# NVIDIA/MinkowskiEngine

Measured on AMD Instinct MI355X. Metric: MinkowskiConvolution fwd+bwd Mpoints/sec (100k-pt 3D, k=3), higher is better.
Workload: dtype f32

## Files before the change

minkowskiengine_amd/csrc/conv.hip:

```cpp
#include "conv_common.hpp"
#include "wgrad_reduce.hpp"

#include <algorithm>
#include <type_traits>
#include <vector>

namespace me {

__host__ __device__ constexpr int stage_ld(int kc) {
  return kc == 96 ? 100 : (kc >= 32 ? kc : kc + 4);
}
__device__ __forceinline__ int stage_swz(int kc, int row) {
  return kc == 96 ? 0 : (kc >= 64 ? (row & 15) : (kc == 32 ? ((row >> 1) & 7) : 0));
}

__host__ __device__ constexpr int conv_lds_bytes(int nc, int kc, int tile_rows, int batch_groups) {
  return (tile_rows + 1) * (nc + kAccPad) * 4 + batch_groups * 16 * (stage_ld(kc) * 4 + 4);
}

template <int R, int KQ, int A_LD, int ACC_LD, int VAR = 0>
__device__ __forceinline__ void mma_groups(const float *__restrict__ a0p, const int (&pofs)[KQ / 4],
                                           const float (&wreg)[KQ], const int32_t *__restrict__ dstp,
                                           float *__restrict__ accp) {
  int d[R];
// ... 1263 lines not shown
  __syncthreads();                                   \
  cm = cw;
    for (;;) {
      ME_WG_STEP(1)
      ME_WG_STEP(2)
      ME_WG_STEP(3)
      ME_WG_STEP(0)
    }
#undef ME_WG_STEP
  } else {
    __builtin_amdgcn_s_setprio(2);
    const int i16 = lane & 15, q = lane >> 4;
    const int cob = blockIdx.z * 4 + wave;
    constexpr int kImage = MB * NB * 4 * 64;
    const int64_t image_stride = (int64_t)gridDim.y * n_cob * kImage;
    float *const image0 = partial + ((int64_t)blockIdx.y * n_cob + min(cob, n_cob - 1)) * kImage + lane;
    f32x4 acc[MB][NB];
    auto zero_acc = [&]() {
#pragma unroll
      for (int m = 0; m < MB; ++m)
#pragma unroll
        for (int n = 0; n < NB; ++n) acc[m][n] = f32x4{0.f, 0.f, 0.f, 0.f};
    };
    auto flush = [&](int k) {
      if (cob < n_cob) {
        float *img = image0 + (int64_t)(range + k) * image_stride;
#pragma unroll
        for (int m = 0; m < MB; ++m)
#pragma unroll
          for (int n = 0; n < NB; ++n)
#pragma unroll
            for (int r = 0; r < 4; ++r) img[((m * NB + n) * 4 + r) * 64] = acc[m][n][r];
      }
    };
    const int frag_row = 4 * q + (i16 >> 2);
    const int frag_col = 4 * (i16 & 3);
    auto multiply = [&](int buf) {
      const __bf16 *bx = s_x + (buf * SP + frag_row) * XLD + frag_col;
      const __bf16 *bd = s_d + (buf * SP + frag_row) * DLD + wave * 16 * NB + frag_col;
#pragma unroll
      for (int ks = 0; ks < KSTEPS; ++ks) {
        bf16x8 a[MB], b[NB];
#pragma unroll
        for (int m = 0; m < MB; ++m) {
          const bf16x4 lo = __builtin_amdgcn_ds_read_tr16_b64_v4bf16((lds_bf16x4 *)(bx + (ks * 32) * XLD + 16 * m));
          const bf16x4 hi = __builtin_amdgcn_ds_read_tr16_b64_v4bf16((lds_bf16x4 *)(bx + (ks * 32 + 16) * XLD + 16 * m));
          a[m] = bf16x8{lo[0], lo[1], lo[2], lo[3], hi[0], hi[1], hi[2], hi[3]};
        }
#pragma unroll
        for (int n = 0; n < NB; ++n) {
          const bf16x4 lo = __builtin_amdgcn_ds_read_tr16_b64_v4bf16((lds_bf16x4 *)(bd + (ks * 32) * DLD + 16 * n));
          const bf16x4 hi = __builtin_amdgcn_ds_read_tr16_b64_v4bf16((lds_bf16x4 *)(bd + (ks * 32 + 16) * DLD + 16 * n));
          b[n] = bf16x8{lo[0], lo[1], lo[2], lo[3], hi[0], hi[1], hi[2], hi[3]};
        }
#pragma unroll
        for (int m = 0; m < MB; ++m)
#pragma unroll
          for (int n = 0; n < NB; ++n) acc[m][n] = __builtin_amdgcn_mfma_f32_16x16x32_bf16(a[m], b[n], acc[m][n], 0, 0, 0);
      }
    };
    Cur cA = first_cur();
    Cur cB = next_cur(cA);
    zero_acc();
    __syncthreads();
    int buf = 0;
    while (cA.cnt > 0) {
      multiply(buf);
      if (cB.cnt == 0 || cB.k != cA.k) {
        flush(cA.k);
        zero_acc();
      }
      __syncthreads();
      buf ^= 1;
      cA = cB;
      cB = next_cur(cB);
    }
    __builtin_amdgcn_s_setprio(0);
  }
}

#endif

template <int NB>
__global__ __launch_bounds__(256, 3) void k_wgrad_f32x3(const float *__restrict__ x, int c_in,
                                                       const float *__restrict__ dy, int c_out,
                                                       const int32_t *__restrict__ in_pairs,
                                                       const int32_t *__restrict__ out_pairs,
                                                       const int64_t *__restrict__ koffs, int volume,
                                                       int64_t n_pairs, int n_ranges, int n_cob,
                                                       float *__restrict__ partial, const WgRangeOrder order) {
  typedef __attribute__((address_space(3))) bf16x4 lds_bf16x4;
  constexpr int MB = 4;
  constexpr int SP = 32;
  constexpr int COB = 64 * NB;
  constexpr int XLD = 64 + kWgStepLd;
  constexpr int DLD = COB + kWgStepLd;
  constexpr int XPL = SP * XLD, DPL = SP * DLD;
  constexpr int XP = SP * 8 / 256;
  constexpr int DP = SP * (COB / 8) / 256;
  static_assert(XP == 1 && DP >= 1, "step size");
  extern __shared__ __attribute__((aligned(16))) char smem[];
  __bf16 *s_x = reinterpret_cast<__bf16 *>(smem);
  __bf16 *s_d = s_x + 3 * XPL;

  const int tid = threadIdx.x;
  const int lane = tid & 63;
  const int wave = __builtin_amdgcn_readfirstlane(tid >> 6);
  const int i16 = lane & 15, q = lane >> 4;
  const int range = order.n > 0 ? (int)order.v[blockIdx.x] : (int)blockIdx.x;
  const int ci0 = blockIdx.y * 64;
  const int cog = blockIdx.z * COB;
  const int cob = blockIdx.z * 4 + wave;
  const int64_t e_lo = n_pairs * range / n_ranges;
  const int64_t e_hi = n_pairs * (range + 1) / n_ranges;
  if (e_lo >= e_hi) return;

  constexpr int kImage = MB * NB * 4 * 64;
  const int64_t image_stride = (int64_t)gridDim.y * n_cob * kImage;
  float *const image0 = partial + ((int64_t)blockIdx.y * n_cob + min(cob, n_cob - 1)) * kImage + lane;

  auto first_offset = [&](int64_t e) {
    int lo = 0, hi = volume;
    while (hi - lo > 1) {
      const int mid = (lo + hi) >> 1;
      if (koffs[mid] <= e) lo = mid; else hi = mid;
    }
    return lo;
  };
  auto step_count = [&](int k, int64_t e) -> int {
    if (e >= e_hi) return 0;
    const int64_t kend = min(koffs[k + 1], e_hi);
    return (int)min((int64_t)SP, kend - e);
  };
  auto advance = [&](int &k, int64_t &e, int cnt) {
    e += cnt;
    if (e < e_hi) {
      while (koffs[k + 1] <= e) ++k;
    }
  };

  int32_t pin = 0, pout = 0;
  f32x4 rx[XP][2], rd[DP][2];
  auto load_idx = [&](int64_t e) {
    const int64_t ec = min(e + lane, n_pairs - 1);
    const int32_t *pi = in_pairs + ec, *po = out_pairs + ec;
    asm volatile("global_load_dword %0, %1, off" : "=v"(pin) : "v"(pi) : "memory");
    asm volatile("global_load_dword %0, %1, off" : "=v"(pout) : "v"(po) : "memory");
  };
  auto load_rows = [&]() {
#pragma unroll
    for (int j = 0; j < XP; ++j) {
      const int idx = j * 256 + tid;
      const int row = idx >> 3;
      const int ch = ci0 + (idx & 7) * 8;
      const int32_t r = __shfl(pin, row, 64);
      const float *p = x + (int64_t)r * c_in + (ch < c_in ? ch : 0);
      asm volatile("global_load_dwordx4 %0, %1, off" : "=v"(rx[j][0]) : "v"(p) : "memory");
      asm volatile("global_load_dwordx4 %0, %1, off offset:16" : "=v"(rx[j][1]) : "v"(p) : "memory");
    }
#pragma unroll
    for (int j = 0; j < DP; ++j) {
      const int idx = j * 256 + tid;
      const int row = idx / (COB / 8);
      const int ch = cog + (idx % (COB / 8)) * 8;
      const int32_t r = __shfl(pout, row, 64);
      const float *p = dy + (int64_t)r * c_out + (ch < c_out ? ch : 0);
      asm volatile("global_load_dwordx4 %0, %1, off" : "=v"(rd[j][0]) : "v"(p) : "memory");
      asm volatile("global_load_dwordx4 %0, %1, off offset:16" : "=v"(rd[j][1]) : "v"(p) : "memory");
    }
  };
  auto wait_rows = [&]() {
    asm volatile("s_waitcnt vmcnt(0)" : "+v"(pin), "+v"(pout));
#pragma unroll
// ... 43 lines not shown
  };

  f32x4 acc[MB][NB];
  auto zero_acc = [&]() {
#pragma unroll
    for (int m = 0; m < MB; ++m)
#pragma unroll
      for (int n = 0; n < NB; ++n) acc[m][n] = f32x4{0.f, 0.f, 0.f, 0.f};
  };
  auto flush = [&](int k) {
    if (cob < n_cob) {
      float *img = image0 + (int64_t)(range + k) * image_stride;
#pragma unroll
      for (int m = 0; m < MB; ++m)
#pragma unroll
        for (int n = 0; n < NB; ++n)
#pragma unroll
          for (int r = 0; r < 4; ++r) img[((m * NB + n) * 4 + r) * 64] = acc[m][n][r];
    }
  };
  const int frag_row = 4 * q + (i16 >> 2);
  const int frag_col = 4 * (i16 & 3);
  auto multiply = [&]() {
    const __bf16 *bx = s_x + frag_row * XLD + frag_col;
    const __bf16 *bd = s_d + frag_row * DLD + wave * 16 * NB + frag_col;
    bf16x8 a[3][MB], b[3][NB];
#pragma unroll
    for (int pl = 0; pl < 3; ++pl) {
#pragma unroll
      for (int m = 0; m < MB; ++m) {
        const bf16x4 lo = __builtin_amdgcn_ds_read_tr16_b64_v4bf16((lds_bf16x4 *)(bx + pl * XPL + 16 * m));
        const bf16x4 hi = __builtin_amdgcn_ds_read_tr16_b64_v4bf16((lds_bf16x4 *)(bx + pl * XPL + 16 * XLD + 16 * m));
        a[pl][m] = bf16x8{lo[0], lo[1], lo[2], lo[3], hi[0], hi[1], hi[2], hi[3]};
      }
#pragma unroll
      for (int n = 0; n < NB; ++n) {
        const bf16x4 lo = __builtin_amdgcn_ds_read_tr16_b64_v4bf16((lds_bf16x4 *)(bd + pl * DPL + 16 * n));
        const bf16x4 hi = __builtin_amdgcn_ds_read_tr16_b64_v4bf16((lds_bf16x4 *)(bd + pl * DPL + 16 * DLD + 16 * n));
        b[pl][n] = bf16x8{lo[0], lo[1], lo[2], lo[3], hi[0], hi[1], hi[2], hi[3]};
      }
    }
    constexpr int XPI[6] = {2, 0, 1, 1, 0, 0};
    constexpr int DPI[6] = {0, 2, 1, 0, 1, 0};
#pragma unroll
    for (int t = 0; t < 6; ++t)
#pragma unroll
      for (int m = 0; m < MB; ++m)
#pragma unroll
        for (int n = 0; n < NB; ++n)
          acc[m][n] = __builtin_amdgcn_mfma_f32_16x16x32_bf16(a[XPI[t]][m], b[DPI[t]][n], acc[m][n], 0, 0, 0);
  };

  int kA = first_offset(e_lo);
  int64_t eA = e_lo;
  int cA = step_count(kA, eA);
  int kB = kA;
  int64_t eB = eA;
  advance(kB, eB, cA);
  int cB = step_count(kB, eB);
  int kC = kB;
  int64_t eC = eB;
  advance(kC, eC, cB);
  int cC = step_count(kC, eC);

  load_idx(eA);
  asm volatile("s_waitcnt vmcnt(0)" : "+v"(pin), "+v"(pout));
  load_rows();
  load_idx(eB);
  zero_acc();
  int pending = -1;
  while (cA > 0) {
    if (pending >= 0) {
      flush(pending);
      zero_acc();
    }
    wait_rows();
    __syncthreads();
    write_lds(cA);
    load_rows();
    load_idx(eC);
    __builtin_amdgcn_sched_barrier(0);
    __syncthreads();
    multiply();
    pending = (cB == 0 || kB != kA) ? kA : -1;
    kA = kB; eA = eB; cA = cB;
    kB = kC; eB = eC; cB = cC;
    advance(kC, eC, cC);
    cC = step_count(kC, eC);
  }
  wait_rows();
  if (pending >= 0) flush(pending);
}

#ifdef ME_DEBUG_VARIANTS
template <int NB, int KSTEPS>
__global__ __launch_bounds__(256, 2) void k_wgrad_lds_f32(const float *__restrict__ x, int c_in,
                                                         const float *__restrict__ dy, int c_out,
                                                      const int32_t *__restrict__ in_pairs,
                                                      const int32_t *__restrict__ out_pairs,
                                                      const int64_t *__restrict__ koffs, int volume,
                                                      int64_t n_pairs, int n_ranges, int n_cob,
                                                      float *__restrict__ partial) {
  constexpr int MB = 4;
  constexpr int SP = 16 * KSTEPS;
  constexpr int COB = 64 * NB;
  constexpr int XLD = 64 + kWgStepLd;
  constexpr int DLD = COB + kWgStepLd;
  constexpr int XP = SP * 16 / 256;
  constexpr int DP = SP * (COB / 4) / 256;
  static_assert(SP <= 64 && XP >= 1, "step size");
  extern __shared__ __attribute__((aligned(16))) char smem[];
  float *s_x = reinterpret_cast<float *>(smem);
  float *s_d = s_x + 2 * SP * XLD;

  const int tid = threadIdx.x;
  const int lane = tid & 63;
  const int wave = __builtin_amdgcn_readfirstlane(tid >> 6);
  const int i16 = lane & 15, q = lane >> 4;
  const int range = blockIdx.x;
  const int ci0 = blockIdx.y * 64;
  const int cog = blockIdx.z * COB;
  const int cob = blockIdx.z * 4 + wave;
  const int64_t e_lo = n_pairs * range / n_ranges;
  const int64_t e_hi = n_pairs * (range + 1) / n_ranges;
  if (e_lo >= e_hi) return;

  constexpr int kImage = MB * NB * 4 * 64;
  const int64_t image_stride = (int64_t)gridDim.y * n_cob * kImage;
  float *const image0 = partial + ((int64_t)blockIdx.y * n_cob + min(cob, n_cob - 1)) * kImage + lane;

  auto first_offset = [&](int64_t e) {
    int lo = 0, hi = volume;
    while (hi - lo > 1) {
      const int mid = (lo + hi) >> 1;
      if (koffs[mid] <= e) lo = mid; else hi = mid;
    }
    return lo;
  };
  auto step_count = [&](int k, int64_t e) -> int {
    if (e >= e_hi) return 0;
    const int64_t kend = min(koffs[k + 1], e_hi);
    return (int)min((int64_t)SP, kend - e);
  };
  auto advance = [&](int &k, int64_t &e, int cnt) {
    e += cnt;
    if (e < e_hi) {
      while (koffs[k + 1] <= e) ++k;
    }
  };

  int32_t pin = 0, pout = 0;
  f32x4 rx[XP], rd[DP];
  auto load_idx = [&](int64_t e) {
    const int64_t ec = min(e + lane, n_pairs - 1);
    const int32_t *pi = in_pairs + ec, *po = out_pairs + ec;
    asm volatile("global_load_dword %0, %1, off" : "=v"(pin) : "v"(pi) : "memory");
    asm volatile("global_load_dword %0, %1, off" : "=v"(pout) : "v"(po) : "memory");
  };
  auto load_rows = [&]() {
#pragma unroll
    for (int j = 0; j < XP; ++j) {
      const int idx = j * 256 + tid;
      const int row = idx >> 4;
      const int ch = ci0 + (idx & 15) * 4;
      const int32_t r = __shfl(pin, row, 64);
      const float *p = x + (int64_t)r * c_in + (ch < c_in ? ch : 0);
// ... 260 lines not shown
                            const int32_t *plan_src, const int32_t *plan_dst, const int32_t *batch_desc,
                            const int32_t *tile_bptr, const int32_t *order, float *dst, int64_t n_tgt,
                            int tile_rows, int batch_groups, hipStream_t stream, bool small = false, bool fuse = false) {
  const int lds = conv_lds_bytes(NC, KC, tile_rows, batch_groups) +
                  (g_conv_variant >= 2048 && g_conv_variant < 3000 ? (g_conv_variant - 2048) * 1024 : 0);
  ME_CHECK(lds <= kLdsBudget, "tile_rows / batch_groups too large for the LDS of one workgroup");
  const bool exact = (c_src % KC) == 0;
  constexpr bool kHasSmall = VAR == 0;
  small = small && kHasSmall;
  typedef void (*kernel_t)(const float *, int, const f32x4 *, int, const int32_t *, const int32_t *, const int32_t *,
                           const int32_t *, const int32_t *, float *, int64_t, int, int);
  kernel_t fn = (small && exact) ? &k_conv_tile_f32<NC, KC, true, VAR, kHasSmall> : &k_conv_tile_f32<NC, KC, false, VAR, false>;
  constexpr bool kHasFuse = VAR == 0 && NC <= 64 && KC <= 64;
  if constexpr (kHasFuse) {
    if (fuse && small) fn = exact ? &k_conv_tile_f32<NC, KC, true, 0, true, true> : &k_conv_tile_f32<NC, KC, false, 0, true, true>;
    else fuse = false;
  } else {
    fuse = false;
  }
  static bool attr_set[6] = {false, false, false, false, false, false};
  const int which = fuse ? 4 + (exact ? 1 : 0) : (small ? 2 : 0) + (exact ? 1 : 0);
  if (lds > 48 * 1024 && !attr_set[which]) {
    ME_HIP(hipFuncSetAttribute(reinterpret_cast<const void *>(fn), hipFuncAttributeMaxDynamicSharedMemorySize,
                               kLdsBudget));
    attr_set[which] = true;
  }
  const dim3 grid((unsigned)ceil_div(n_tgt, tile_rows), (unsigned)slabs);
  hipLaunchKernelGGL(fn, grid, dim3(NC * 4), (size_t)lds, stream, src, c_src, reinterpret_cast<const f32x4 *>(wp), c_dst,
                     plan_src, plan_dst, batch_desc, tile_bptr, order, dst, n_tgt, tile_rows, batch_groups);
  ME_LAUNCH_CHECK();
  return 0;
}

template <int NC, int CBW, int KCH>
static int launch_conv_tile_dma(const float *src, int c_src, const float *wp, int c_dst, const int32_t *plan_src,
                                const int32_t *plan_dst, const int32_t *batch_desc, const int32_t *tile_bptr,
                                const int32_t *order, float *dst, int64_t n_tgt, int tile_rows, int batch_groups,
                                hipStream_t stream) {
  const int lds = conv_dma_lds_bytes(NC, KCH, tile_rows, batch_groups);
  ME_CHECK(lds <= kLdsBudget, "tile_rows / batch_groups too large for the LDS of one workgroup (LDS-DMA kernel)");
  typedef void (*kernel_t)(const float *, int, const f32x4 *, int, const int32_t *, const int32_t *, const int32_t *,
                           const int32_t *, const int32_t *, float *, int64_t, int, int);
  kernel_t fn = &k_conv_tile_dma_f32<NC, CBW, KCH, 0>;
  const int code = g_conv_variant % 100;
  if (code == 16) fn = &k_conv_tile_dma_f32<NC, CBW, KCH, 16>;
  if constexpr (NC == 128 && CBW == 2) {
    if (code == 2) fn = &k_conv_tile_dma_f32<NC, CBW, KCH, 2>;
    if (code == 4) fn = &k_conv_tile_dma_f32<NC, CBW, KCH, 4>;
    if (code == 32) fn = &k_conv_tile_dma_f32<NC, CBW, KCH, 32>;
    if (code == 64) fn = &k_conv_tile_dma_f32<NC, CBW, KCH, 64>;
    if (code == 99) fn = &k_conv_tile_dma_f32<NC, CBW, KCH, 16 + 2 + 4 + 32 + 64>;
    if (code == 98) fn = &k_conv_tile_dma_f32<NC, CBW, KCH, 512>;
  }
  ME_HIP(hipFuncSetAttribute(reinterpret_cast<const void *>(fn), hipFuncAttributeMaxDynamicSharedMemorySize,
                             kLdsBudget));
  const dim3 grid((unsigned)ceil_div(n_tgt, tile_rows), (unsigned)(c_dst / NC));
  hipLaunchKernelGGL(fn, grid, dim3(NC / CBW * 4), (size_t)lds, stream, src, c_src,
                     reinterpret_cast<const f32x4 *>(wp), c_dst, plan_src, plan_dst, batch_desc, tile_bptr, order, dst,
                     n_tgt, tile_rows, batch_groups);
  ME_LAUNCH_CHECK();
  return 0;
}

struct ConvDmaShape {
  int nc, cbw, kch;
};
static ConvDmaShape conv_dma_shape(int c_src, int c_dst) {
  ConvDmaShape z{0, 0, 0};
  if (g_conv_variant < 3000 || g_conv_variant >= 3400) return z;
  if (c_src % 64 != 0 || c_dst % 64 != 0) return z;
  const int family = g_conv_variant / 100;
  if (family == 30) {
    if (g_conv_variant == 3064) return ConvDmaShape{64, 1, 1};
    return c_dst % 128 == 0 ? ConvDmaShape{128, 1, 1} : ConvDmaShape{64, 1, 1};
  }
  if (c_dst % 128 == 0) return ConvDmaShape{128, 2, 1};
  if (c_src % 128 == 0) return ConvDmaShape{64, 1, 2};
  return ConvDmaShape{64, 1, 1};
}

int g_wgrad_depth = 0;
int g_wgrad_wgs_per_cu = 0;
int g_wgrad_order = 0;

struct WgradGeom {
  int nb;
  int n_cib;
  int n_cob;
  int waves;
  int gz;
  int64_t ranges;
  int64_t slot_floats;
};

static WgradGeom wgrad_geom(int64_t n_pairs, int64_t volume, int c_in, int c_out) {
  WgradGeom g;
  g.nb = c_out <= 64 ? 1 : (c_out <= 128 ? 2 : 4);
  if (g_wgrad_depth >= 100) g.nb = g_wgrad_depth / 100;
  g.n_cib = (int)ceil_div(c_in, 16 * kWgMB);
  g.n_cob = (int)ceil_div(c_out, 16 * g.nb);
  g.waves = g.n_cob < 4 ? g.n_cob : 4;
  g.gz = (int)ceil_div(g.n_cob, g.waves);
  const int wpc = g_wgrad_wgs_per_cu > 0 ? g_wgrad_wgs_per_cu : 3;
  int64_t r = ceil_div((int64_t)device_cu_count() * wpc, (int64_t)g.n_cib * g.gz);
  if (r > n_pairs / 64) r = n_pairs / 64;
  if (r < 1) r = 1;
  g.ranges = r;
  g.slot_floats = (int64_t)g.n_cib * g.n_cob * (kWgMB * g.nb * 4 * 64);
  (void)volume;
  return g;
}

int g_wgrad_ws = 0;
int g_wgrad_mb = 0;

static int wgrad_bf16_mb(int c_in, int c_out) {
  if (g_wgrad_mb == 4 || g_wgrad_mb == 8) return (g_wgrad_mb == 8 && c_out > 64) ? 8 : 4;
  return (c_in >= 192 && c_out > 64) ? 8 : 4;
}

static WgradGeom wgrad_geom_staged(int64_t n_pairs, int c_in, int c_out, int wpc_default = 2, int mb = kWgMB) {
  WgradGeom g;
  g.nb = c_out <= 64 ? 1 : 2;
  g.n_cib = (int)ceil_div(c_in, 16 * mb);
  g.n_cob = (int)ceil_div(c_out, 16 * g.nb);
  g.waves = 4;
  g.gz = (int)ceil_div(g.n_cob, 4);
  const int wpc = g_wgrad_wgs_per_cu > 0 ? g_wgrad_wgs_per_cu : (g.n_cib == 3 ? 3 : wpc_default);
  int64_t r = ceil_div((int64_t)device_cu_count() * wpc, (int64_t)g.n_cib * g.gz);
  if (r > n_pairs / 64) r = n_pairs / 64;
  if (r < 1) r = 1;
  g.ranges = r;
  g.slot_floats = (int64_t)g.n_cib * g.n_cob * (mb * g.nb * 4 * 64);
  return g;
}

template <int NB, int KSTEPS, int MB = kWgMB>
static int launch_wgrad_bf16(const WgradGeom &g, const __bf16 *x, int c_in, const __bf16 *dy, int c_out,
                             const int32_t *in_pairs, const int32_t *out_pairs, const int64_t *k_offsets_dev,
                             int volume, int64_t n_pairs, float *partial, hipStream_t stream) {
  constexpr int SP = 32 * KSTEPS;
  const int lds = 2 * SP * ((16 * MB + kWgStepLd) + (64 * NB + kWgStepLd)) * 2;
  auto fn = &k_wgrad_bf16<NB, KSTEPS, MB>;
  static bool attr_set = false;
  if (lds > 32 * 1024 && !attr_set) {
    ME_HIP(hipFuncSetAttribute(reinterpret_cast<const void *>(fn), hipFuncAttributeMaxDynamicSharedMemorySize,
                               kLdsBudget));
    attr_set = true;
  }
  const dim3 grid((unsigned)g.ranges, (unsigned)g.n_cib, (unsigned)g.gz);
#ifdef ME_DEBUG_VARIANTS
  if (g_wgrad_ws != 0) {
    auto ws = g_wgrad_ws == 2 ? &k_wgrad_bf16_ws<NB, KSTEPS, MB, 2> : &k_wgrad_bf16_ws<NB, KSTEPS, MB, (MB == 8 ? 2 : 4)>;
    static bool ws_attr[2] = {false, false};
    if (lds > 32 * 1024 && !ws_attr[g_wgrad_ws == 2]) {
      ME_HIP(hipFuncSetAttribute(reinterpret_cast<const void *>(ws), hipFuncAttributeMaxDynamicSharedMemorySize, kLdsBudget));
      ws_attr[g_wgrad_ws == 2] = true;
    }
    hipLaunchKernelGGL(ws, grid, dim3(512), (size_t)lds, stream, x, c_in, dy, c_out, in_pairs, out_pairs, k_offsets_dev,
                       volume, n_pairs, (int)g.ranges, g.n_cob, partial);
    ME_LAUNCH_CHECK();
    return 0;
  }
#endif
  hipLaunchKernelGGL(fn, grid, dim3(256), (size_t)lds, stream, x, c_in, dy, c_out, in_pairs,
                     out_pairs, k_offsets_dev, volume, n_pairs, (int)g.ranges, g.n_cob, partial);
  ME_LAUNCH_CHECK();
  return 0;
}

#ifdef ME_DEBUG_VARIANTS
template <int NB, int KSTEPS>
static int launch_wgrad_lds_f32(const WgradGeom &g, const float *x, int c_in, const float *dy, int c_out,
                                const int32_t *in_pairs, const int32_t *out_pairs, const int64_t *k_offsets_dev,
                                int volume, int64_t n_pairs, float *partial, hipStream_t stream) {
  constexpr int SP = 16 * KSTEPS;
  const int lds = 2 * SP * ((64 + kWgStepLd) + (64 * NB + kWgStepLd)) * 4;
  static bool attr_set = false;
  if (lds > 32 * 1024 && !attr_set) {
    ME_HIP(hipFuncSetAttribute(reinterpret_cast<const void *>(&k_wgrad_lds_f32<NB, KSTEPS>),
                               hipFuncAttributeMaxDynamicSharedMemorySize, kLdsBudget));
    attr_set = true;
  }
  const dim3 grid((unsigned)g.ranges, (unsigned)g.n_cib, (unsigned)g.gz);
  hipLaunchKernelGGL((k_wgrad_lds_f32<NB, KSTEPS>), grid, dim3(256), (size_t)lds, stream, x, c_in, dy, c_out,
                     in_pairs, out_pairs, k_offsets_dev, volume, n_pairs, (int)g.ranges, g.n_cob, partial);
  ME_LAUNCH_CHECK();
  return 0;
}
#endif

template <int NB>
static int launch_wgrad_f32x3(const WgradGeom &g, const float *x, int c_in, const float *dy, int c_out,
                              const int32_t *in_pairs, const int32_t *out_pairs, const int64_t *k_offsets_dev,
                              int volume, int64_t n_pairs, float *partial, const WgRangeOrder &order,
                              hipStream_t stream) {
  const int lds = 3 * 32 * ((64 + kWgStepLd) + (64 * NB + kWgStepLd)) * 2;
  const dim3 grid((unsigned)g.ranges, (unsigned)g.n_cib, (unsigned)g.gz);
  hipLaunchKernelGGL((k_wgrad_f32x3<NB>), grid, dim3(256), (size_t)lds, stream, x, c_in, dy, c_out, in_pairs,
                     out_pairs, k_offsets_dev, volume, n_pairs, (int)g.ranges, g.n_cob, partial, order);
  ME_LAUNCH_CHECK();
  return 0;
}

static bool wgrad_use_split(int c_in, int c_out) {
  if (g_wgrad_depth == -3 || (c_in % 8) != 0 || (c_out % 8) != 0) return false;
  if (g_wgrad_depth == -4) return true;
  return g_wgrad_depth == 0 && c_in >= 32 && c_out >= 32;
}

bool wgrad_split_tail(const int64_t *k_offsets, const int64_t *k_offsets_dev, int64_t volume, int c_in, int c_out,
                      const void *workspace, float *grad_w, WgTail *tail) {
  if (!wgrad_use_split(c_in, c_out) || volume < 1 || volume > 65535) return false;
  const int64_t n_pairs = k_offsets[volume];
  const WgradGeom g = wgrad_geom_staged(n_pairs, c_in, c_out, 3);
  tail->r = WgReduceArgs{reinterpret_cast<const float *>(workspace), k_offsets_dev, grad_w, n_pairs > 0 ? n_pairs : 1,
                         (int)volume, (int)g.ranges, g.n_cib, g.n_cob, c_in, c_out};
  tail->nb = g.nb;
  tail->n_tiles = 0;
  return true;
}

}

using namespace me;

static WgRangeOrder wgrad_range_order(const int64_t *k_offsets, int64_t volume, int64_t n_pairs, int64_t ranges,
                                      int64_t wgs_per_range) {
  WgRangeOrder o;
  o.n = 0;
  if (g_wgrad_order < 0 || ranges < 64 || ranges > kWgMaxOrder || wgs_per_range != 1 || volume < 2) return o;
  struct Item {
    double f;
    int r;
  };
  std::vector<Item> items((size_t)ranges);
  int k = 0;
  for (int64_t r = 0; r < ranges; ++r) {
    const int64_t e = wgrad_range_begin(r, n_pairs, ranges);
    while (k + 1 < volume && k_offsets[k + 1] <= e) ++k;
    const int64_t len = k_offsets[k + 1] - k_offsets[k];
    items[(size_t)r] = {len > 0 ? (double)(e - k_offsets[k]) / (double)len : 0.0, (int)r};
  }
  std::stable_sort(items.begin(), items.end(), [](const Item &a, const Item &b) { return a.f < b.f; });
  constexpr int kXcds = 8, kGroup = 32;
  std::vector<std::vector<int>> per_xcd(kXcds);
  for (int64_t i = 0; i < ranges; ++i) per_xcd[(size_t)((i / kGroup) % kXcds)].push_back(items[(size_t)i].r);
  std::vector<int> assigned((size_t)ranges, -1), spill;
  for (int x = 0; x < kXcds; ++x) {
    for (size_t i = 0; i < per_xcd[(size_t)x].size(); ++i) {
      const int64_t b = (int64_t)i * kXcds + x;
      if (b < ranges) assigned[(size_t)b] = per_xcd[(size_t)x][i];
      else spill.push_back(per_xcd[(size_t)x][i]);
    }
  }
  size_t sp = 0;
  for (int64_t b = 0; b < ranges; ++b)
    if (assigned[(size_t)b] < 0) assigned[(size_t)b] = spill[sp++];
  o.n = (int)ranges;
  for (int64_t b = 0; b < ranges; ++b) o.v[b] = (uint16_t)assigned[(size_t)b];
  return o;
}

template <typename T>
static int wgrad_launch(const T *x, int64_t n_in, int32_t c_in, const T *dy, int64_t n_out, int32_t c_out,
                        const int32_t *in_pairs, const int32_t *out_pairs, const int64_t *k_offsets,
                        const int64_t *k_offsets_dev, int64_t volume, float *grad_w, void *workspace,
                        int64_t workspace_bytes, hipStream_t stream) {
  ME_CHECK(volume >= 1 && volume <= 65535, "kernel volume out of range");
  ME_CHECK(c_in > 0 && c_out > 0, "channel counts must be positive");
  ME_CHECK((uintptr_t)x % 16 == 0 && (uintptr_t)dy % 16 == 0, "feature pointers must be 16-byte aligned");
  ME_CHECK(workspace_bytes >= me_conv_wgrad_workspace_bytes(k_offsets, volume, c_in, c_out),
           "workspace too small");
  const int64_t n_pairs = k_offsets[volume];
  const WgradGeom g = wgrad_geom(n_pairs, volume, c_in, c_out);
  float *partial = reinterpret_cast<float *>(workspace);
  const int depth = (g_wgrad_depth > 0 && g_wgrad_depth % 100 > 0) ? g_wgrad_depth % 100 : (g.nb == 4 ? 8 : 4);
  if (n_pairs > 0) {
    const dim3 grid((unsigned)g.ranges, (unsigned)g.n_cib, (unsigned)g.gz);
    const dim3 block(64 * g.waves);
    const bool vec = (c_in % kWgMB) == 0 && (c_out % g.nb) == 0;
    const int64_t lim = 1ll << 32;
    const bool small = n_in > 0 && n_out > 0 && n_in < (1 << 24) && n_out < (1 << 24) &&
                       n_in * c_in * (int64_t)sizeof(T) < lim && n_out * c_out * (int64_t)sizeof(T) < lim &&
                       g_conv_variant != 6;
    const WgRangeOrder order = wgrad_range_order(k_offsets, volume, n_pairs, g.ranges, (int64_t)g.n_cib * g.gz);
#define ME_WGRAD_LAUNCH(NBV, DV)                                                                                 \
  do {                                                                                                           \
    if (vec && small)                                                                                            \
      hipLaunchKernelGGL((k_wgrad_f32<T, NBV, DV, true, true>), grid, block, 0, stream, x, c_in, dy, c_out,      \
                         in_pairs, out_pairs, k_offsets_dev, (int)volume, n_pairs, (int)g.ranges, g.n_cob,       \
// ... 138 lines not shown
    if (v.kc == 96) ME_CONV_CASE(64, 96);
    if (v.kc == 64) ME_CONV_CASE(64, 64);
    if (v.kc == 32) ME_CONV_CASE(64, 32);
    ME_CONV_CASE(64, 16);
  }
#undef ME_CONV_CASE
#undef ME_CONV_ARGS
}

int me_conv_target_f32(const float *src, int64_t n_src, int32_t c_src, const float *wp, int64_t volume,
                       int32_t c_dst, const int32_t *plan_src, const int32_t *plan_dst,
                       const int32_t *batch_desc, const int32_t *tile_bptr, const int32_t *order, float *dst,
                       int64_t n_tgt, int32_t tile_rows, int32_t batch_groups, void *stream) {
  return conv_target_f32(src, n_src, c_src, wp, volume, c_dst, plan_src, plan_dst, batch_desc, tile_bptr, order, dst,
                         n_tgt, tile_rows, batch_groups, stream, false);
}

int me_conv_target_f32_fused(const float *src, int64_t n_src, int32_t c_src, const float *wp, int64_t volume,
                             int32_t c_dst, const int32_t *plan_src, const int32_t *plan_dst,
                             const int32_t *batch_desc, const int32_t *tile_bptr, const int32_t *order, float *dst,
                             int64_t n_tgt, int32_t tile_rows, int32_t batch_groups, void *stream) {
  return conv_target_f32(src, n_src, c_src, wp, volume, c_dst, plan_src, plan_dst, batch_desc, tile_bptr, order, dst,
                         n_tgt, tile_rows, batch_groups, stream, true);
}

int32_t me_debug_variants_compiled(void) {
#ifdef ME_DEBUG_VARIANTS
  return 1;
#else
  return 0;
#endif
}

int me_debug_set_conv_variant(int variant) {
#ifndef ME_DEBUG_VARIANTS
  const bool ok = variant == 0 || variant == 6 || variant == 7 || variant == 9 || variant == 30 || variant == 31;
  ME_CHECK(ok, "this conv variant needs a -DME_DEBUG_VARIANTS build of libme_amd.so (tuning / ablation kernels)");
#endif
  g_conv_variant = variant;
  return 0;
}

int me_debug_conv_timing(uint64_t *out8, int32_t reset) {
  unsigned long long h[8] = {0, 0, 0, 0, 0, 0, 0, 0};
  if (out8 != nullptr) {
    ME_HIP(hipMemcpyFromSymbol(h, HIP_SYMBOL(d_conv_timing), sizeof(h)));
    for (int i = 0; i < 8; ++i) out8[i] = h[i];
  }
  if (reset) {
    unsigned long long z[8] = {0, 0, 0, 0, 0, 0, 0, 0};
    ME_HIP(hipMemcpyToSymbol(HIP_SYMBOL(d_conv_timing), z, sizeof(z)));
  }
  return 0;
}


int me_transpose_kernel_f32(const float *w, int64_t volume, int32_t c_in, int32_t c_out, float *wt,
                            void *stream_) {
  hipStream_t stream = (hipStream_t)stream_;
  ME_CHECK(volume >= 1 && volume <= 65535, "kernel volume out of range");
  const dim3 grid((unsigned)ceil_div(c_out, 32), (unsigned)ceil_div(c_in, 32), (unsigned)volume);
  hipLaunchKernelGGL(k_transpose_kernel, grid, dim3(256), 0, stream, w, volume, c_in, c_out, wt);
  ME_LAUNCH_CHECK();
  return 0;
}

int64_t me_conv_wgrad_workspace_bytes(const int64_t *k_offsets, int64_t volume, int32_t c_in, int32_t c_out) {
  if (volume < 1 || c_in <= 0 || c_out <= 0) return 256;
  const WgradGeom g = wgrad_geom(k_offsets[volume], volume, c_in, c_out);
  const WgradGeom h = wgrad_geom_staged(k_offsets[volume], c_in, c_out, 3);
  const int64_t a = (g.ranges + volume) * g.slot_floats, b = (h.ranges + volume) * h.slot_floats;
  return align_up((a > b ? a : b) * 4, 256);
}

void me_debug_set_wgrad_order(int mode) { g_wgrad_order = mode; }
void me_debug_set_wgrad_mb(int mb) { g_wgrad_mb = mb; }
void me_debug_set_wgrad_ws(int mode) { g_wgrad_ws = mode; }

void me_debug_set_wgrad_config(int depth, int wgs_per_cu) {
  g_wgrad_depth = depth;
  g_wgrad_wgs_per_cu = wgs_per_cu;
}

static int wgrad_split_partials(const float *x, int32_t c_in, const float *dy, int32_t c_out, const int32_t *in_pairs,
                                const int32_t *out_pairs, const int64_t *k_offsets, const int64_t *k_offsets_dev,
                                int64_t volume, void *workspace, int64_t workspace_bytes, hipStream_t stream,
                                WgradGeom *geom) {
  ME_CHECK(volume >= 1 && volume <= 65535, "kernel volume out of range");
  ME_CHECK((uintptr_t)x % 16 == 0 && (uintptr_t)dy % 16 == 0, "feature pointers must be 16-byte aligned");
  ME_CHECK(workspace_bytes >= me_conv_wgrad_workspace_bytes(k_offsets, volume, c_in, c_out), "workspace too small");
  const int64_t n_pairs = k_offsets[volume];
  const WgradGeom g = wgrad_geom_staged(n_pairs, c_in, c_out, 3);
  float *partial = reinterpret_cast<float *>(workspace);
  *geom = g;
  if (n_pairs <= 0) return 0;
  const WgRangeOrder order = wgrad_range_order(k_offsets, volume, n_pairs, g.ranges, (int64_t)g.n_cib * g.gz);
  return g.nb == 1 ? launch_wgrad_f32x3<1>(g, x, c_in, dy, c_out, in_pairs, out_pairs, k_offsets_dev, (int)volume,
                                           n_pairs, partial, order, stream)
                   : launch_wgrad_f32x3<2>(g, x, c_in, dy, c_out, in_pairs, out_pairs, k_offsets_dev, (int)volume,
                                           n_pairs, partial, order, stream);
}

int32_t me_conv_wgrad_is_split_f32(int32_t c_in, int32_t c_out) { return wgrad_use_split(c_in, c_out) ? 1 : 0; }

int me_conv_wgrad_partials_f32(const float *x, int64_t n_in, int32_t c_in, const float *dy, int64_t n_out, int32_t c_out,
                               const int32_t *in_pairs, const int32_t *out_pairs, const int64_t *k_offsets,
                               const int64_t *k_offsets_dev, int64_t volume, void *workspace, int64_t workspace_bytes,
                               void *stream_) {
  (void)n_in;
  (void)n_out;
  ME_CHECK(wgrad_use_split(c_in, c_out), "not a split weight gradient (me_conv_wgrad_is_split_f32)");
  WgradGeom g;
  return wgrad_split_partials(x, c_in, dy, c_out, in_pairs, out_pairs, k_offsets, k_offsets_dev, volume, workspace,
                              workspace_bytes, (hipStream_t)stream_, &g);
}

int me_conv_wgrad_f32(const float *x, int64_t n_in, int32_t c_in, const float *dy, int64_t n_out, int32_t c_out,
                      const int32_t *in_pairs,
                      const int32_t *out_pairs, const int64_t *k_offsets, const int64_t *k_offsets_dev,
                      int64_t volume, float *grad_w, void *workspace, int64_t workspace_bytes,
                      void *stream_) {
  hipStream_t stream = (hipStream_t)stream_;
  if (wgrad_use_split(c_in, c_out)) {
    WgradGeom g;
    const int rc = wgrad_split_partials(x, c_in, dy, c_out, in_pairs, out_pairs, k_offsets, k_offsets_dev, volume,
                                        workspace, workspace_bytes, stream, &g);
    if (rc != 0) return rc;
    const float *partial = reinterpret_cast<const float *>(workspace);
    const int64_t n_pairs = k_offsets[volume];
    const dim3 rgrid((unsigned)ceil_div(g.slot_floats, 256), (unsigned)volume);
    if (g.nb == 1)
      hipLaunchKernelGGL((k_wgrad_reduce<1, true>), rgrid, dim3(64 * kWgReducePhases), 0, stream, partial, k_offsets_dev,
                         (int)volume, n_pairs > 0 ? n_pairs : 1, (int)g.ranges, g.n_cib, g.n_cob, c_in, c_out, grad_w);
    else
      hipLaunchKernelGGL((k_wgrad_reduce<2, true>), rgrid, dim3(64 * kWgReducePhases), 0, stream, partial, k_offsets_dev,
                         (int)volume, n_pairs > 0 ? n_pairs : 1, (int)g.ranges, g.n_cib, g.n_cob, c_in, c_out, grad_w);
    ME_LAUNCH_CHECK();
    return 0;
  }
#ifndef ME_DEBUG_VARIANTS
  return wgrad_launch<float>(x, n_in, c_in, dy, n_out, c_out, in_pairs, out_pairs, k_offsets, k_offsets_dev, volume, grad_w,
                             workspace, workspace_bytes, stream);
#else
  if ((c_in % 4) != 0 || (c_out % 4) != 0 || g_wgrad_depth != -2)
    return wgrad_launch<float>(x, n_in, c_in, dy, n_out, c_out, in_pairs, out_pairs, k_offsets, k_offsets_dev, volume, grad_w,
                               workspace, workspace_bytes, stream);
  ME_CHECK(volume >= 1 && volume <= 65535, "kernel volume out of range");
  ME_CHECK(c_in > 0 && c_out > 0, "channel counts must be positive");
  ME_CHECK((uintptr_t)x % 16 == 0 && (uintptr_t)dy % 16 == 0, "feature pointers must be 16-byte aligned");
  ME_CHECK(workspace_bytes >= me_conv_wgrad_workspace_bytes(k_offsets, volume, c_in, c_out), "workspace too small");
  const int64_t n_pairs = k_offsets[volume];
  const WgradGeom g = wgrad_geom_staged(n_pairs, c_in, c_out);
  float *partial = reinterpret_cast<float *>(workspace);
  if (n_pairs > 0) {
    int rc;
    if (g.nb == 1)
      rc = launch_wgrad_lds_f32<1, 2>(g, x, c_in, dy, c_out, in_pairs, out_pairs, k_offsets_dev, (int)volume, n_pairs,
                                      partial, stream);
    else
      rc = launch_wgrad_lds_f32<2, 2>(g, x, c_in, dy, c_out, in_pairs, out_pairs, k_offsets_dev, (int)volume, n_pairs,
                                      partial, stream);
    if (rc != 0) return rc;
  }
  const dim3 rgrid((unsigned)ceil_div(g.slot_floats, 256), (unsigned)volume);
  if (g.nb == 1)
    hipLaunchKernelGGL((k_wgrad_reduce<1, true>), rgrid, dim3(64 * kWgReducePhases), 0, stream, partial, k_offsets_dev, (int)volume,
                       n_pairs > 0 ? n_pairs : 1, (int)g.ranges, g.n_cib, g.n_cob, c_in, c_out, grad_w);
  else
    hipLaunchKernelGGL((k_wgrad_reduce<2, true>), rgrid, dim3(64 * kWgReducePhases), 0, stream, partial, k_offsets_dev, (int)volume,
                       n_pairs > 0 ? n_pairs : 1, (int)g.ranges, g.n_cib, g.n_cob, c_in, c_out, grad_w);
  ME_LAUNCH_CHECK();
  return 0;
#endif
}

}

extern "C" {

int64_t me_conv_wgrad_workspace_bytes_bf16(const int64_t *k_offsets, int64_t volume, int32_t c_in, int32_t c_out) {
  if (volume < 1 || c_in <= 0 || c_out <= 0) return 256;
  const WgradGeom g4 = wgrad_geom_staged(k_offsets[volume], c_in, c_out, 2, 4);
  const WgradGeom g8 = wgrad_geom_staged(k_offsets[volume], c_in, c_out, 2, 8);
  const int64_t a4 = align_up((g4.ranges + volume) * g4.slot_floats * 4, 256);
  const int64_t a8 = align_up((g8.ranges + volume) * g8.slot_floats * 4, 256);
  const int64_t a = a4 > a8 ? a4 : a8;
  const int64_t b = me_conv_wgrad_workspace_bytes(k_offsets, volume, c_in, c_out);
  return a > b ? a : b;
}

int me_conv_wgrad_bf16(const uint16_t *x_, int64_t n_in, int32_t c_in, const uint16_t *dy_, int64_t n_out,
                       int32_t c_out, const int32_t *in_pairs,
                       const int32_t *out_pairs, const int64_t *k_offsets, const int64_t *k_offsets_dev,
                       int64_t volume, float *grad_w, void *workspace, int64_t workspace_bytes,
                       void *stream_) {
  hipStream_t stream = (hipStream_t)stream_;
  const __bf16 *x = reinterpret_cast<const __bf16 *>(x_);
  const __bf16 *dy = reinterpret_cast<const __bf16 *>(dy_);
  ME_CHECK(workspace_bytes >= me_conv_wgrad_workspace_bytes_bf16(k_offsets, volume, c_in, c_out),
           "workspace too small");
  if ((c_in % 8) != 0 || (c_out % 8) != 0 || g_wgrad_depth < 0)
    return wgrad_launch<__bf16>(x, n_in, c_in, dy, n_out, c_out, in_pairs, out_pairs, k_offsets, k_offsets_dev, volume, grad_w,
                                workspace, workspace_bytes, stream);
  ME_CHECK(volume >= 1 && volume <= 65535, "kernel volume out of range");
  ME_CHECK((uintptr_t)x % 16 == 0 && (uintptr_t)dy % 16 == 0, "feature pointers must be 16-byte aligned");
  const int64_t n_pairs = k_offsets[volume];
  const int mb = wgrad_bf16_mb(c_in, c_out);
  const WgradGeom g = wgrad_geom_staged(n_pairs, c_in, c_out, 2, mb);
// ... 61 lines not shown
```

Baseline: 340.6.

## Load dy fragments directly into MFMA B registers, skip LDS staging in wgrad

Adds a new split-bf16x3 weight-gradient kernel that gathers dy values for each lane's MFMA B fragment straight from global memory into registers and splits them there. Only x goes through LDS, double-buffered, so the dy staging buffer and its LDS traffic disappear and the LDS footprint shrinks. When n_out*c_out fits in 32 bits, dy loads use a 32-bit offset with a scalar base instead of 64-bit pointers. The old staged kernel is kept behind debug flags. The cost is many more scalar dword gathers and higher register pressure per thread.

```diff
diff --git a/minkowskiengine_amd/csrc/conv.hip b/minkowskiengine_amd/csrc/conv.hip
--- a/minkowskiengine_amd/csrc/conv.hip
+++ b/minkowskiengine_amd/csrc/conv.hip
@@ -1369,13 +1369,13 @@
 #endif
 
 template <int NB>
-__global__ __launch_bounds__(256, 3) void k_wgrad_f32x3(const float *__restrict__ x, int c_in,
-                                                       const float *__restrict__ dy, int c_out,
-                                                       const int32_t *__restrict__ in_pairs,
-                                                       const int32_t *__restrict__ out_pairs,
-                                                       const int64_t *__restrict__ koffs, int volume,
-                                                       int64_t n_pairs, int n_ranges, int n_cob,
-                                                       float *__restrict__ partial, const WgRangeOrder order) {
+__global__ __launch_bounds__(256, 3) void k_wgrad_f32x3_staged(const float *__restrict__ x, int c_in,
+                                                              const float *__restrict__ dy, int c_out,
+                                                              const int32_t *__restrict__ in_pairs,
+                                                              const int32_t *__restrict__ out_pairs,
+                                                              const int64_t *__restrict__ koffs, int volume,
+                                                              int64_t n_pairs, int n_ranges, int n_cob,
+                                                              float *__restrict__ partial, const WgRangeOrder order) {
   typedef __attribute__((address_space(3))) bf16x4 lds_bf16x4;
   constexpr int MB = 4;
   constexpr int SP = 32;
@@ -1585,6 +1585,249 @@
     __builtin_amdgcn_sched_barrier(0);
     __syncthreads();
     multiply();
+    pending = (cB == 0 || kB != kA) ? kA : -1;
+    kA = kB; eA = eB; cA = cB;
+    kB = kC; eB = eC; cB = cC;
+    advance(kC, eC, cC);
+    cC = step_count(kC, eC);
+  }
+  wait_rows();
+  if (pending >= 0) flush(pending);
+}
+
+template <int NB, bool OFF32>
+__global__ __launch_bounds__(256, 3) void k_wgrad_f32x3(const float *__restrict__ x, int c_in,
+                                                       const float *__restrict__ dy, int c_out,
+                                                       const int32_t *__restrict__ in_pairs,
+                                                       const int32_t *__restrict__ out_pairs,
+                                                       const int64_t *__restrict__ koffs, int volume,
+                                                       int64_t n_pairs, int n_ranges, int n_cob,
+                                                       float *__restrict__ partial, const WgRangeOrder order) {
+  typedef __attribute__((address_space(3))) bf16x4 lds_bf16x4;
+  constexpr int MB = 4;
+  constexpr int SP = 32;
+  constexpr int COB = 64 * NB;
+  constexpr int XLD = 64 + kWgStepLd;
+  constexpr int XPL = SP * XLD;
+  constexpr int XBUF = 3 * XPL;
+  static_assert(SP * 8 == 256, "one 8-channel x piece per thread and step");
+  extern __shared__ __attribute__((aligned(16))) char smem[];
+  __bf16 *s_x = reinterpret_cast<__bf16 *>(smem);
+
+  const int tid = threadIdx.x;
+  const int lane = tid & 63;
+  const int wave = __builtin_amdgcn_readfirstlane(tid >> 6);
+  const int i16 = lane & 15, q = lane >> 4;
+  const int range = order.n > 0 ? (int)order.v[blockIdx.x] : (int)blockIdx.x;
+  const int ci0 = blockIdx.y * 64;
+  const int cog = blockIdx.z * COB;
+  const int cob = blockIdx.z * 4 + wave;
+  const int64_t e_lo = n_pairs * range / n_ranges;
+  const int64_t e_hi = n_pairs * (range + 1) / n_ranges;
+  if (e_lo >= e_hi) return;
+
+  constexpr int kImage = MB * NB * 4 * 64;
+  const int64_t image_stride = (int64_t)gridDim.y * n_cob * kImage;
+  float *const image0 = partial + ((int64_t)blockIdx.y * n_cob + min(cob, n_cob - 1)) * kImage + lane;
+
+  auto first_offset = [&](int64_t e) {
+    int lo = 0, hi = volume;
+    while (hi - lo > 1) {
+      const int mid = (lo + hi) >> 1;
+      if (koffs[mid] <= e) lo = mid; else hi = mid;
+    }
+    return lo;
+  };
+  auto step_count = [&](int k, int64_t e) -> int {
+    if (e >= e_hi) return 0;
+    const int64_t kend = min(koffs[k + 1], e_hi);
+    return (int)min((int64_t)SP, kend - e);
+  };
+  auto advance = [&](int &k, int64_t &e, int cnt) {
+    e += cnt;
+    if (e < e_hi) {
+      while (koffs[k + 1] <= e) ++k;
+    }
+  };
+
+  const int xrow = tid >> 3;
+  const int xch = ci0 + (tid & 7) * 8;
+  const bool xok = xch < c_in;
+  int dcol[NB];
+  bool dok[NB];
+  bool dfull = true;
+#pragma unroll
+  for (int n = 0; n < NB; ++n) {
+    const int col = cog + 16 * NB * wave + 16 * n + i16;
+    dok[n] = col < c_out;
+    dcol[n] = dok[n] ? col : 0;
+    dfull = dfull && dok[n];
+  }
+  const bool full_cols = __all(dfull);
+  auto slot_pair = [&](int s) { return (s < 4 ? 0 : 12) + 4 * q + s; };
+
+  int32_t pin = 0, pout = 0;
+  f32x4 rx[2];
+  float rd[NB][8];
+  auto load_idx = [&](int64_t e) {
+    const int64_t ec = min(e + lane, n_pairs - 1);
+    const int32_t *pi = in_pairs + ec, *po = out_pairs + ec;
+    asm volatile("global_load_dword %0, %1, off" : "=v"(pin) : "v"(pi) : "memory");
+    asm volatile("global_load_dword %0, %1, off" : "=v"(pout) : "v"(po) : "memory");
+  };
+  auto load_rows = [&]() {
+    {
+      const int32_t r = __shfl(pin, xrow, 64);
+      const float *p = x + (int64_t)r * c_in + (xok ? xch : 0);
+      asm volatile("global_load_dwordx4 %0, %1, off" : "=v"(rx[0]) : "v"(p) : "memory");
+      asm volatile("global_load_dwordx4 %0, %1, off offset:16" : "=v"(rx[1]) : "v"(p) : "memory");
+    }
+#pragma unroll
+    for (int s = 0; s < 8; ++s) {
+      const int32_t r = __shfl(pout, slot_pair(s), 64);
+      if (OFF32) {
+        const uint32_t ro = (uint32_t)r * (uint32_t)c_out;
+#pragma unroll
+        for (int n = 0; n < NB; ++n) {
+          const uint32_t off = (ro + (uint32_t)dcol[n]) * 4u;
+          asm volatile("global_load_dword %0, %1, %2" : "=v"(rd[n][s]) : "v"(off), "s"(dy) : "memory");
+        }
+      } else {
+        const float *pr = dy + (int64_t)r * c_out;
+#pragma unroll
+        for (int n = 0; n < NB; ++n) {
+          const float *p = pr + dcol[n];
+          asm volatile("global_load_dword %0, %1, off" : "=v"(rd[n][s]) : "v"(p) : "memory");
+        }
+      }
+    }
+  };
+  auto wait_rows = [&]() {
+    asm volatile("s_waitcnt vmcnt(0)" : "+v"(pin), "+v"(pout), "+v"(rx[0]), "+v"(rx[1]));
+#pragma unroll
+    for (int n = 0; n < NB; ++n)
+      asm volatile("s_waitcnt vmcnt(0)"
+                   : "+v"(rd[n][0]), "+v"(rd[n][1]), "+v"(rd[n][2]), "+v"(rd[n][3]), "+v"(rd[n][4]), "+v"(rd[n][5]),
+                     "+v"(rd[n][6]), "+v"(rd[n][7]));
+  };
+  auto split_step = [&](int cnt, int buf, bf16x8 (&b)[3][NB], auto mask, auto fix) {
+    constexpr bool MASK = decltype(mask)::value;
+    constexpr bool FIX = decltype(fix)::value;
+    const u32x4 zero = {0u, 0u, 0u, 0u};
+    uint32_t flag = 0u;
+    {
+      const bool ok = xrow < cnt && xok;
+      u32x4 p1, p2, p3;
+      if (FIX) split3_fix<false>(rx[0], rx[1], p1, p2, p3);
+      else split3_raw(rx[0], rx[1], p1, p2, p3);
+      if (ok) flag = split3_flag(flag, p3);
+      __bf16 *o = s_x + buf * XBUF + xrow * XLD + (tid & 7) * 8;
+      *reinterpret_cast<u32x4 *>(o) = ok ? p1 : zero;
+      *reinterpret_cast<u32x4 *>(o + XPL) = ok ? p2 : zero;
+      *reinterpret_cast<u32x4 *>(o + 2 * XPL) = ok ? p3 : zero;
+    }
+#pragma unroll
+    for (int n = 0; n < NB; ++n) {
+      float v[8];
+#pragma unroll
+      for (int s = 0; s < 8; ++s) v[s] = (!MASK || (dok[n] && slot_pair(s) < cnt)) ? rd[n][s] : 0.f;
+      const f32x4 lo = {v[0], v[1], v[2], v[3]}, hi = {v[4], v[5], v[6], v[7]};
+      u32x4 p1, p2, p3;
+      if (FIX) split3_fix<true>(lo, hi, p1, p2, p3);
+      else split3_raw(lo, hi, p1, p2, p3);
+      flag = split3_flag(flag, p3);
+      b[0][n] = __builtin_bit_cast(bf16x8, p1);
+      b[1][n] = __builtin_bit_cast(bf16x8, p2);
+      b[2][n] = __builtin_bit_cast(bf16x8, p3);
+    }
+    return flag;
+  };
+  auto split_rows = [&](int cnt, int buf, bf16x8 (&b)[3][NB]) {
+    if (cnt == SP && full_cols) {
+      const uint32_t flag = split_step(cnt, buf, b, std::false_type{}, std::false_type{});
+      if (__builtin_expect(__any(split3_suspect(flag)), 0)) split_step(cnt, buf, b, std::false_type{}, std::true_type{});
+    } else {
+      const uint32_t flag = split_step(cnt, buf, b, std::true_type{}, std::false_type{});
+      if (__builtin_expect(__any(split3_suspect(flag)), 0)) split_step(cnt, buf, b, std::true_type{}, std::true_type{});
+    }
+  };
+
+  f32x4 acc[MB][NB];
+  auto zero_acc = [&]() {
+#pragma unroll
+    for (int m = 0; m < MB; ++m)
+#pragma unroll
+      for (int n = 0; n < NB; ++n) acc[m][n] = f32x4{0.f, 0.f, 0.f, 0.f};
+  };
+  auto flush = [&](int k) {
+    if (cob < n_cob) {
+      float *img = image0 + (int64_t)(range + k) * image_stride;
+#pragma unroll
+      for (int m = 0; m < MB; ++m)
+#pragma unroll
+        for (int n = 0; n < NB; ++n)
+#pragma unroll
+          for (int r = 0; r < 4; ++r) img[((m * NB + n) * 4 + r) * 64] = acc[m][n][r];
+    }
+  };
+  const int frag_row = 4 * q + (i16 >> 2);
+  const int frag_col = 4 * (i16 & 3);
+  auto multiply = [&](int buf, const bf16x8 (&b)[3][NB]) {
+    const __bf16 *bx = s_x + buf * XBUF + frag_row * XLD + frag_col;
+    bf16x8 a[3][MB];
+#pragma unroll
+    for (int pl = 0; pl < 3; ++pl) {
+#pragma unroll
+      for (int m = 0; m < MB; ++m) {
+        const bf16x4 lo = __builtin_amdgcn_ds_read_tr16_b64_v4bf16((lds_bf16x4 *)(bx + pl * XPL + 16 * m));
+        const bf16x4 hi = __builtin_amdgcn_ds_read_tr16_b64_v4bf16((lds_bf16x4 *)(bx + pl * XPL + 16 * XLD + 16 * m));
+        a[pl][m] = bf16x8{lo[0], lo[1], lo[2], lo[3], hi[0], hi[1], hi[2], hi[3]};
+      }
+    }
+    constexpr int XPI[6] = {2, 0, 1, 1, 0, 0};
+    constexpr int DPI[6] = {0, 2, 1, 0, 1, 0};
+#pragma unroll
+    for (int t = 0; t < 6; ++t)
+#pragma unroll
+      for (int m = 0; m < MB; ++m)
+#pragma unroll
+        for (int n = 0; n < NB; ++n)
+          acc[m][n] = __builtin_amdgcn_mfma_f32_16x16x32_bf16(a[XPI[t]][m], b[DPI[t]][n], acc[m][n], 0, 0, 0);
+  };
+
+  int kA = first_offset(e_lo);
+  int64_t eA = e_lo;
+  int cA = step_count(kA, eA);
+  int kB = kA;
+  int64_t eB = eA;
+  advance(kB, eB, cA);
+  int cB = step_count(kB, eB);
+  int kC = kB;
+  int64_t eC = eB;
+  advance(kC, eC, cB);
+  int cC = step_count(kC, eC);
+
+  load_idx(eA);
+  asm volatile("s_waitcnt vmcnt(0)" : "+v"(pin), "+v"(pout));
+  load_rows();
+  load_idx(eB);
+  zero_acc();
+  int pending = -1;
+  int buf = 0;
+  while (cA > 0) {
+    if (pending >= 0) {
+      flush(pending);
+      zero_acc();
+    }
+    bf16x8 b[3][NB];
+    wait_rows();
+    split_rows(cA, buf, b);
+    load_rows();
+    load_idx(eC);
+    __builtin_amdgcn_sched_barrier(0);
+    __syncthreads();
+    multiply(buf, b);
+    buf ^= 1;
     pending = (cB == 0 || kB != kA) ? kA : -1;
     kA = kB; eA = eB; cA = cB;
     kB = kC; eB = eC; cB = cC;
@@ -2011,6 +2254,7 @@
 int g_wgrad_depth = 0;
 int g_wgrad_wgs_per_cu = 0;
 int g_wgrad_order = 0;
+static bool wgrad_split_staged() { return g_wgrad_depth == -5 || g_wgrad_depth == -6; }
 
 struct WgradGeom {
   int nb;
@@ -2120,22 +2364,34 @@
 #endif
 
 template <int NB>
-static int launch_wgrad_f32x3(const WgradGeom &g, const float *x, int c_in, const float *dy, int c_out,
+static int launch_wgrad_f32x3(const WgradGeom &g, const float *x, int c_in, const float *dy, int64_t n_out, int c_out,
                               const int32_t *in_pairs, const int32_t *out_pairs, const int64_t *k_offsets_dev,
                               int volume, int64_t n_pairs, float *partial, const WgRangeOrder &order,
                               hipStream_t stream) {
-  const int lds = 3 * 32 * ((64 + kWgStepLd) + (64 * NB + kWgStepLd)) * 2;
   const dim3 grid((unsigned)g.ranges, (unsigned)g.n_cib, (unsigned)g.gz);
-  hipLaunchKernelGGL((k_wgrad_f32x3<NB>), grid, dim3(256), (size_t)lds, stream, x, c_in, dy, c_out, in_pairs,
-                     out_pairs, k_offsets_dev, volume, n_pairs, (int)g.ranges, g.n_cob, partial, order);
+  if (wgrad_split_staged()) {
+    const int lds = 3 * 32 * ((64 + kWgStepLd) + (64 * NB + kWgStepLd)) * 2;
+    hipLaunchKernelGGL((k_wgrad_f32x3_staged<NB>), grid, dim3(256), (size_t)lds, stream, x, c_in, dy, c_out, in_pairs,
+                       out_pairs, k_offsets_dev, volume, n_pairs, (int)g.ranges, g.n_cob, partial, order);
+    ME_LAUNCH_CHECK();
+    return 0;
+  }
+  const int lds = 2 * 3 * 32 * (64 + kWgStepLd) * 2;
+  const bool off32 = n_out > 0 && (uint64_t)n_out * (uint64_t)c_out * 4u < (1ull << 32);
+  if (off32)
+    hipLaunchKernelGGL((k_wgrad_f32x3<NB, true>), grid, dim3(256), (size_t)lds, stream, x, c_in, dy, c_out, in_pairs,
+                       out_pairs, k_offsets_dev, volume, n_pairs, (int)g.ranges, g.n_cob, partial, order);
+  else
+    hipLaunchKernelGGL((k_wgrad_f32x3<NB, false>), grid, dim3(256), (size_t)lds, stream, x, c_in, dy, c_out, in_pairs,
+                       out_pairs, k_offsets_dev, volume, n_pairs, (int)g.ranges, g.n_cob, partial, order);
   ME_LAUNCH_CHECK();
   return 0;
 }
 
 static bool wgrad_use_split(int c_in, int c_out) {
   if (g_wgrad_depth == -3 || (c_in % 8) != 0 || (c_out % 8) != 0) return false;
-  if (g_wgrad_depth == -4) return true;
-  return g_wgrad_depth == 0 && c_in >= 32 && c_out >= 32;
+  if (g_wgrad_depth == -4 || g_wgrad_depth == -6) return true;
+  return (g_wgrad_depth == 0 || g_wgrad_depth == -5) && c_in >= 32 && c_out >= 32;
 }
 
 bool wgrad_split_tail(const int64_t *k_offsets, const int64_t *k_offsets_dev, int64_t volume, int c_in, int c_out,
@@ -2440,7 +2696,8 @@
   g_wgrad_wgs_per_cu = wgs_per_cu;
 }
 
-static int wgrad_split_partials(const float *x, int32_t c_in, const float *dy, int32_t c_out, const int32_t *in_pairs,
+static int wgrad_split_partials(const float *x, int32_t c_in, const float *dy, int64_t n_out, int32_t c_out,
+                                const int32_t *in_pairs,
                                 const int32_t *out_pairs, const int64_t *k_offsets, const int64_t *k_offsets_dev,
                                 int64_t volume, void *workspace, int64_t workspace_bytes, hipStream_t stream,
                                 WgradGeom *geom) {
@@ -2453,9 +2710,9 @@
   *geom = g;
   if (n_pairs <= 0) return 0;
   const WgRangeOrder order = wgrad_range_order(k_offsets, volume, n_pairs, g.ranges, (int64_t)g.n_cib * g.gz);
-  return g.nb == 1 ? launch_wgrad_f32x3<1>(g, x, c_in, dy, c_out, in_pairs, out_pairs, k_offsets_dev, (int)volume,
+  return g.nb == 1 ? launch_wgrad_f32x3<1>(g, x, c_in, dy, n_out, c_out, in_pairs, out_pairs, k_offsets_dev, (int)volume,
                                            n_pairs, partial, order, stream)
-                   : launch_wgrad_f32x3<2>(g, x, c_in, dy, c_out, in_pairs, out_pairs, k_offsets_dev, (int)volume,
+                   : launch_wgrad_f32x3<2>(g, x, c_in, dy, n_out, c_out, in_pairs, out_pairs, k_offsets_dev, (int)volume,
                                            n_pairs, partial, order, stream);
 }
 
@@ -2466,10 +2723,9 @@
                                const int64_t *k_offsets_dev, int64_t volume, void *workspace, int64_t workspace_bytes,
                                void *stream_) {
   (void)n_in;
-  (void)n_out;
   ME_CHECK(wgrad_use_split(c_in, c_out), "not a split weight gradient (me_conv_wgrad_is_split_f32)");
   WgradGeom g;
-  return wgrad_split_partials(x, c_in, dy, c_out, in_pairs, out_pairs, k_offsets, k_offsets_dev, volume, workspace,
+  return wgrad_split_partials(x, c_in, dy, n_out, c_out, in_pairs, out_pairs, k_offsets, k_offsets_dev, volume, workspace,
                               workspace_bytes, (hipStream_t)stream_, &g);
 }
 
@@ -2481,7 +2737,7 @@
   hipStream_t stream = (hipStream_t)stream_;
   if (wgrad_use_split(c_in, c_out)) {
     WgradGeom g;
-    const int rc = wgrad_split_partials(x, c_in, dy, c_out, in_pairs, out_pairs, k_offsets, k_offsets_dev, volume,
+    const int rc = wgrad_split_partials(x, c_in, dy, n_out, c_out, in_pairs, out_pairs, k_offsets, k_offsets_dev, volume,
                                         workspace, workspace_bytes, stream, &g);
     if (rc != 0) return rc;
     const float *partial = reinterpret_cast<const float *>(workspace);
```

After: 342.7 (median of 6 runs). Within noise of the previous version (+0.6%).
